# TrondVQ/UncertaintyQuantification-SleepApnea-1DCNN

Hardware: AMD Instinct MI355X
Metric: 30s-windows/sec for MCD T=50 & DE M=8 inference at 1/2/4/8 MI355X (higher is better)
Workload: dtype fp32; 1 GPU; global_batch=16384, seq_len=60, parallelism=dp1, mcd_passes=50, de_members=8, bn_mode_mcd=batch

## Files before the change

uncertaintyquantification_sleepapnea_1dcnn_amd/csrc/x3_api.h:

```cpp
#pragma once
#include <hip/hip_runtime_api.h>

#include <cstdint>

#include "x3_args.h"
#include "x3_geo.h"

namespace apneauq {
x3::LayerInfo x3_layer_info(int layer);
hipError_t x3_launch_layer(int layer, const x3::LayerArgs& A, int grid, bool dense_rows, hipStream_t stream);
hipError_t x3_launch_l1(const x3::L1Args& A, hipStream_t stream);
hipError_t x3_launch_aff(const x3::AffArgs& A, hipStream_t stream);
hipError_t x3_launch_head(const x3::HeadArgs& A, hipStream_t stream);
}
```

uncertaintyquantification_sleepapnea_1dcnn_amd/csrc/x3_bindings.cpp:

```cpp
#include "arch_tables.h"
#include "bind_util.h"
#include "x3_api.h"

namespace {
using namespace apneauq::bind;
constexpr auto& kCh = apneauq::arch::C;
constexpr auto& kKs = apneauq::arch::KS;

int num_cus(const at::Tensor& t) {
  int n = 0;
  check(hipDeviceGetAttribute(&n, hipDeviceAttributeMultiprocessorCount, t.device().index()), "hipDeviceGetAttribute");
  return n > 0 ? n : 256;
}

void x3_layer(int64_t layer, const at::Tensor& in, at::Tensor& out, const at::Tensor& wfrag, int64_t w_gstride,
              const at::Tensor& bias, const at::Tensor& wscale, int64_t p_gstride, const at::Tensor& aff_in,
              int64_t aff_gstride, const c10::optional<at::Tensor>& stats, int64_t n_win, int64_t groups,
              bool in_shared, int64_t thr_in, int64_t thr_out, int64_t seed, int64_t pass_base,
              int64_t window_offset, int64_t grid, const c10::optional<at::Tensor>& smax_in,
              const c10::optional<at::Tensor>& amax_in, const c10::optional<at::Tensor>& smax_out,
              const c10::optional<at::Tensor>& gscale_in, bool sign_in, bool sign_out, bool dense_rows) {
  TORCH_CHECK(layer >= 1 && layer <= 5, "x3_layer: layer must be 1..5 (block 2..6)");
  TORCH_CHECK(n_win >= 1 && groups >= 1, "x3_layer: empty launch");
  const int cin = kCh[layer], cout = kCh[layer + 1], ks = kKs[layer];
  const int64_t samples = n_win * groups, samples_in = in_shared ? n_win : samples;
  const apneauq::x3::LayerInfo info = apneauq::x3_layer_info((int)layer);
  TORCH_CHECK(!dense_rows || info.has_dense, "x3_layer: layer ", layer, " has no dense-row kernel");
  TORCH_CHECK(!dense_rows || n_win < (int64_t(1) << 24), "x3_layer: too many windows for dense rows");
  const int64_t tpg = apneauq::x3::tiles_per_group<int64_t>(dense_rows, n_win, info.S);
  TORCH_CHECK(tpg * groups < (int64_t(1) << 31), "x3_layer: too many tiles");
  const int64_t wgroups = w_gstride ? groups : 1, pgroups = p_gstride ? groups : 1;
  need(in, at::kFloat, samples_in * 60 * cin, "x3_layer: in");
  need(out, at::kFloat, layer == 5 ? samples * 2 * cout : samples * 60 * cout, "x3_layer: out");
  const int64_t frag = (int64_t)(cin / 32) * ks * (cout / 16) * 128;
  TORCH_CHECK(w_gstride == 0 || w_gstride == frag, "x3_layer: w_gstride must be 0 or ", frag);
  need(wfrag, at::kHalf, wgroups * frag * 8, "x3_layer: wfrag");
  TORCH_CHECK(p_gstride == 0 || p_gstride == cout, "x3_layer: p_gstride must be 0 or ", cout);
  need(bias, at::kFloat, pgroups * cout, "x3_layer: bias");
  need(wscale, at::kFloat, pgroups, "x3_layer: wscale");
  TORCH_CHECK(aff_gstride == 0 || aff_gstride == 2 * cin, "x3_layer: aff_gstride must be 0 or ", 2 * cin);
  need(aff_in, at::kFloat, (aff_gstride ? groups : 1) * 2 * cin, "x3_layer: aff_in");
  double* st = nullptr;
  if (stats.has_value()) {
// ... 39 lines not shown
  A.tiles_per_group = (int)tpg;
  A.total_tiles = (int)(tpg * groups);
  A.in_shared = in_shared ? 1 : 0;
  TORCH_CHECK(!(sign_in && in_shared), "x3_layer: the shared block-1 output carries no masks");
  TORCH_CHECK(!(sign_out && layer == 5), "x3_layer: block 6 reduces its masked output in place");
  A.sign_in = sign_in ? 1 : 0;
  A.sign_out = sign_out ? 1 : 0;
  A.thr_in = (unsigned)thr_in;
  A.thr_out = (unsigned)thr_out;
  A.layer = (int)layer;
  A.pass_base = (unsigned)pass_base;
  A.window_offset = (unsigned)window_offset;
  A.seed = (unsigned long long)seed;
  int g = grid > 0 ? (int)grid : num_cus(in) * info.WPC;
  if (g > A.total_tiles) g = A.total_tiles;
  check(apneauq::x3_launch_layer((int)layer, A, g, dense_rows, cur_stream()), "x3_layer");
}

void x3_l1(const at::Tensor& x, const at::Tensor& w, const at::Tensor& b, at::Tensor& out,
           const c10::optional<at::Tensor>& stats, int64_t n_win, int64_t groups, const c10::optional<at::Tensor>& smax) {
  TORCH_CHECK(n_win >= 1 && groups >= 1, "x3_l1: empty launch");
  need(x, at::kFloat, n_win * 60 * 4, "x3_l1: x");
  need(w, at::kFloat, groups * 7 * 4 * 128, "x3_l1: w");
  need(b, at::kFloat, groups * 128, "x3_l1: b");
  need(out, at::kFloat, groups * n_win * 60 * 128, "x3_l1: out");
  double* st = nullptr;
  if (stats.has_value()) {
    need(*stats, at::kDouble, groups * apneauq::x3::kStatSlots * 2 * 128, "x3_l1: stats");
    st = stats->data_ptr<double>();
  }
  unsigned* smp = nullptr;
// ... 55 lines not shown
  TORCH_CHECK(aff_gstride == 0 || aff_gstride == 2 * C, "x3_head: aff_gstride");
  TORCH_CHECK(p_gstride == 0 || p_gstride == C, "x3_head: p_gstride");
  need(sums, at::kFloat, samples * 2 * C, "x3_head: sums");
  need(aff, at::kFloat, (aff_gstride ? groups : 1) * 2 * C, "x3_head: aff");
  need(dw, at::kFloat, (p_gstride ? groups : 1) * C, "x3_head: dense w");
  need(db, at::kFloat, p_gstride ? groups : 1, "x3_head: dense b");
  need(out, at::kFloat, samples, "x3_head: out");
  const at::DeviceGuard guard(sums.device());
  apneauq::x3::HeadArgs A{sums.data_ptr<float>(), aff.data_ptr<float>(), dw.data_ptr<float>(), db.data_ptr<float>(),
                          out.data_ptr<float>(), C, (int)n_win, (int)samples, (int)aff_gstride, (int)p_gstride,
                          logits ? 1 : 0};
  check(apneauq::x3_launch_head(A, cur_stream()), "x3_head");
}

bool x3_has_dense(int64_t layer) { return apneauq::x3_layer_info((int)layer).has_dense; }

}

TORCH_LIBRARY_FRAGMENT(apneauq, m) {
  m.def("x3_layer(int layer, Tensor input, Tensor(a!) out, Tensor wfrag, int w_gstride, Tensor bias, Tensor wscale, "
        "int p_gstride, Tensor aff_in, int aff_gstride, Tensor(b!)? stats, int n_win, int groups, bool in_shared, "
        "int thr_in, int thr_out, int seed, int pass_base, int window_offset, int grid, Tensor? smax_in=None, "
        "Tensor? amax_in=None, Tensor(c!)? smax_out=None, Tensor? gscale_in=None, bool sign_in=False, bool sign_out=False, "
        "bool dense_rows=False) -> ()");
  m.def("x3_l1(Tensor x, Tensor w, Tensor b, Tensor(a!) out, Tensor(b!)? stats, int n_win, int groups, "
        "Tensor(c!)? smax=None) -> ()");
  m.def("x3_aff(Tensor? stats, Tensor gamma, Tensor beta, Tensor(a!) mmean, Tensor(b!) mvar, Tensor(c!) aff, int C, "
        "int groups, int p_gstride, bool update, int repeat, float inv_count, float eps, float momentum, float dsc, "
        "Tensor(d!)? amax=None, Tensor(e!)? gscale=None, bool running=False) -> ()");
  m.def("x3_head(Tensor sums, Tensor aff, int aff_gstride, Tensor dw, Tensor db, int p_gstride, Tensor(a!) out, "
        "int n_win, int groups, bool logits) -> ()");
  m.def("x3_has_dense(int layer) -> bool", &x3_has_dense);
}

TORCH_LIBRARY_IMPL(apneauq, CUDA, m) {
  m.impl("x3_layer", &x3_layer);
  m.impl("x3_l1", &x3_l1);
  m.impl("x3_head", &x3_head);
  m.impl("x3_aff", &x3_aff);
}
```

uncertaintyquantification_sleepapnea_1dcnn_amd/csrc/x3_geo.h:

```cpp
#pragma once

#include "x3_dense_map.h"

#ifndef __host__
#define APNEAUQ_X3_GEO_PLAIN 1
#define __host__
#define __device__
#endif

namespace apneauq {
namespace x3 {

constexpr int kStagers = 4;
constexpr int kL = 60, kSR = 64, kHalo = 4;
__host__ __device__ constexpr int row_bytes(int ck) { return 4 * ck + 32; }
__host__ __device__ constexpr int lds_rows(int S) { return kHalo + S * kSR + kHalo; }
__host__ __device__ constexpr int buf_bytes(int S, int ck) { return lds_rows(S) * row_bytes(ck); }
__host__ __device__ constexpr int tab_rows(int S, int ks) { return kSR * S + (ks - 1); }
__host__ __device__ constexpr int mask_tab_bytes(int S, int cout) { return kSR * S * (cout / 16) * 2; }
__host__ __device__ constexpr bool mask_tab_layer(int cin, int cout, int ks, int lw, bool dense_rows) {
  return dense_rows && lw > 0 && cin == 96 && cout == 256 && ks == 9;
}

template <int NW, int WPC>
constexpr int waves_per_eu() { return NW * WPC > 8 ? (NW * WPC + 3) / 4 : NW * WPC <= 4 ? 1 : 2; }
constexpr int loaders(int lw) { return lw > 0 ? lw : 0; }
constexpr int dense_lw(int lw, int wm, int wn) { return lw > 0 ? lw : -(wm * wn); }

struct Geo {
  int g, w0, wf, off, rows_left;
};

template <typename I>
__host__ __device__ constexpr I tiles_per_group(bool dense_rows, I n_win, int S) {
  return dense_rows ? (I)dense::tiles(n_win, kSR * S) : (n_win + S - 1) / S;
}
// ... 17 lines not shown
  static constexpr int kRowB = row_bytes(CK), NQ = CK / 32, kQ = CK / 4;
  static constexpr int PAD = (KS - 1) / 2, kRows = kSR * S;
  static_assert(!DENSE || (!PS && !LAST), "dense rows: batch-moment blocks 2..5 only");
  static_assert(kThreads <= 1024, "workgroup size");
  static constexpr int kBufB = DENSE ? dense::lds_rows(kRows) * kRowB : buf_bytes(S, CK);
  static constexpr int kValidRows = DENSE ? kRows : S * kL, kUnits = kValidRows * kQ;
  static constexpr int SW = LW > 0 ? LW : LW < 0 ? (-LW < NW ? -LW : NW) : (kStagers < NW ? kStagers : NW);
  static constexpr int kSBase = LW > 0 ? NWM * 64 : 0;
  static constexpr int kST = SW * 64;
  static constexpr int kMainU = (kUnits + kST - 1) / kST, kNU = kMainU + (DENSE ? 1 : 0);
  static constexpr int kEdgeWaves = (2 * PAD * kQ + 63) / 64;
  static_assert(!DENSE || (kUnits % kST == 0 && kEdgeWaves <= SW), "dense rows: whole staging steps per tile");
  static_assert(kST % kQ == 0 && (CK == 32 || CK == 64), "a staging thread keeps one channel quad");
  static constexpr int NCH = CIN / CK, NCTA = COUT / 16, NCT = NCTA / WN, NRT = 4 * S / WM;
  static constexpr int NSTEP = NCH * NQ * KS;
  static constexpr int RG = NCT >= 4                       ? 1
                            : (NCT >= 3 && NCT * NRT > 16) ? 1
                            : NCT == 1                     ? 4
                                                           : 2;
  static constexpr bool BDB = NCT * NRT <= 24 && RG < 4;
  static_assert(NRT % RG == 0, "row-tile groups");
  static constexpr long long FRAG_STEP = (long long)NCTA * 128;
  static_assert(CIN % CK == 0 && COUT % 16 == 0, "channel tiling");
  static_assert(NCTA % WN == 0 && (4 * S) % WM == 0, "wave tiling");
  static_assert(NRT % 4 == 0, "whole 64-row sample slots per wave row (epilogue keys, block 6 sums)");
  static_assert(S <= 8, "packed per-sample exponents");
  static constexpr int kSP = (S + 3) / 4;

  static constexpr int kTabRows = tab_rows(S, KS);
  static_assert(!DENSE || NCH >= 2, "row tables: a tile's tables are written one chunk of the same workgroup ahead");
  static constexpr bool kMaskTab = mask_tab_layer(CIN, COUT, KS, LW, DENSE);
  static constexpr int kMtRowW = COUT / 16, kMtT = kMaskTab ? kST / kRows : 1, kMtW = kMtRowW / kMtT;
  static constexpr int kMtPhase = (kMtW + (NCH > 1 ? NCH - 2 : 0)) / (NCH > 1 ? NCH - 1 : 1);
  static_assert(!kMaskTab || NCH >= 2, "mask table: written in the chunk iterations ahead of the tile's last");
  static_assert(!kMaskTab || (kST % kRows == 0 && kMtRowW % kMtT == 0), "mask table: whole words per loader thread");

// ... 28 lines not shown
#define APNEAUQ_X3_LAYERS(X)                            \
  X(1, 128, 192, 5, 4, 2, 4, false, -8, 0, 32, 1, true) \
  X(2, 192, 224, 3, 2, 1, 7, false, 4, 4, 64, 1, true)  \
  X(3, 224, 96, 7, 4, 2, 2, false, 4, 4, 32, 1, true)   \
  X(4, 96, 256, 9, 2, 1, 8, false, 4, 4, 32, 1, true)   \
  X(5, 256, 96, 9, 4, 2, 2, true, 4, 4, 64, 1, false)
#endif

namespace apneauq {
namespace x3 {

struct LayerInfo {
  int S, WPC;
  bool has_dense;
  int lds_ps, lds_batch, lds_dense;
};
template <bool HAVE, int CIN, int COUT, int KS, int S, int WM, int WN, int LW, int CK, int WPC>
constexpr int dense_lds_bytes() {
  if constexpr (HAVE) {
    return Cfg<CIN, COUT, KS, S, WM, WN, false, dense_lw(LW, WM, WN), CK, WPC, false, true>::bytes;
  } else {
    return 0;
  }
}
constexpr LayerInfo layer_info(int layer) {
#define APNEAUQ_X3_INFO(L, CI, CO, K, S, WM, WN, LAST, LW, LWB, CK, WPC, DENSE)                              \
  if (layer == L)                                                                                            \
    return LayerInfo{S, WPC, DENSE && !LAST, Cfg<CI, CO, K, S, WM, WN, LAST, LW, CK, WPC, true>::bytes,      \
                     Cfg<CI, CO, K, S, WM, WN, LAST, LWB, CK, WPC, false>::bytes,                            \
                     dense_lds_bytes<DENSE && !LAST, CI, CO, K, S, WM, WN, LWB, CK, WPC>()};
  APNEAUQ_X3_LAYERS(APNEAUQ_X3_INFO)
#undef APNEAUQ_X3_INFO
  return LayerInfo{0, 1, false, 0, 0, 0};
}

}
}

#ifdef APNEAUQ_X3_GEO_PLAIN
#undef __host__
#undef __device__
#undef APNEAUQ_X3_GEO_PLAIN
#endif
```

uncertaintyquantification_sleepapnea_1dcnn_amd/csrc/x3_layers.hip:

```cpp
#include "common.h"
#include "f16x3.h"
#include "x3_api.h"
#include "x3_dense_map.h"
#include "x3_geo.h"

namespace apneauq {
namespace x3 {

__device__ __forceinline__ int sample_prescale(unsigned rmax_bits, const float* amax) {
  return prescale_exp(__builtin_fmaf(amax[0], __uint_as_float(rmax_bits), amax[1]));
}

template <typename T>
__device__ __forceinline__ T gld(const void* p) {
  return *(const __attribute__((address_space(1))) T*)(p);
}

__device__ __forceinline__ int opaque_tid() {
  int t = threadIdx.x;
  asm volatile("" : "+v"(t));
  return t;
}

__device__ __forceinline__ void lds_barrier() {
  __builtin_amdgcn_fence(__ATOMIC_RELEASE, "workgroup", "local");
  __builtin_amdgcn_s_barrier();
  __builtin_amdgcn_fence(__ATOMIC_ACQUIRE, "workgroup", "local");
}

template <int CIN, int COUT, int KS, int S, int WM, int WN, bool LAST, int LW, int CK, int WPC, bool PS, bool DENSE = false>
__global__ __launch_bounds__((WM * WN + loaders(LW)) * 64, (waves_per_eu<WM * WN + loaders(LW), WPC>())) void layer_kernel(
    const LayerArgs A) {
  extern __shared__ __attribute__((aligned(16))) char smem[];
  using C = Cfg<CIN, COUT, KS, S, WM, WN, LAST, LW, CK, WPC, PS, DENSE>;
  constexpr int NWM = C::NWM, kThreads = C::kThreads, kCK = CK, kRowB = C::kRowB, NQ = C::NQ, kQ = C::kQ;
  constexpr int PAD = C::PAD, kRows = C::kRows, kS = S, kBufB = C::kBufB, kValidRows = C::kValidRows;
  constexpr int SW = C::SW, kSBase = C::kSBase, kST = C::kST, kMainU = C::kMainU, kNU = C::kNU;
  constexpr int NCH = C::NCH, NCT = C::NCT, NRT = C::NRT, NSTEP = C::NSTEP, RG = C::RG, kSP = C::kSP;
  constexpr bool BDB = C::BDB;
  constexpr long long FRAG_STEP = C::FRAG_STEP;
  constexpr int kTabRows = C::kTabRows;
  constexpr bool kMaskTab = C::kMaskTab;
  constexpr bool kBiasHoist = DENSE;
  constexpr int kMtRowW = C::kMtRowW, kMtT = C::kMtT, kMtW = C::kMtW, kMtPhase = C::kMtPhase;
  double* st = reinterpret_cast<double*>(smem + C::st);
  float* wsc = reinterpret_cast<float*>(smem + C::wsc);
  unsigned* ektab = reinterpret_cast<unsigned*>(smem + C::ektab);
  uint2* stab = reinterpret_cast<uint2*>(smem + C::stab);
  unsigned short* mtab = reinterpret_cast<unsigned short*>(smem + C::mtab);
// ... 405 lines not shown
            atomicAdd(&st[COUT + co0 + e], (double)b);
          }
        }
      }
    }
    if (track) {
#pragma unroll
      for (int q = 0; q < NRT / 4; ++q) {
        const float mq = wave_max(mxs[q]);
        const int w = w0 + (rt0 >> 2) + q;
        if (lane == 0 && w < A.n_win) atomicMax(A.smax_out + (long long)g * A.n_win + w, __float_as_uint(mq));
      }
    }
  };

  auto flush_stats = [&](int g) {
    __syncthreads();
    if (A.stats != nullptr) {
      double* dst = A.stats + ((long long)g * kStatSlots + slot) * 2 * COUT;
      for (int i = DENSE ? opaque_tid() : tid; i < 2 * COUT; i += kThreads) {
        atomicAdd(dst + i, st[i]);
        st[i] = 0.0;
      }
    }
    __syncthreads();
  };

  for (int i = tid; i < C::st / 16; i += kThreads) reinterpret_cast<f32x4*>(smem)[i] = f32x4{0.f, 0.f, 0.f, 0.f};
  for (int i = tid; i < 2 * COUT; i += kThreads) st[i] = 0.0;
  if (DENSE && stager) write_tables(t_begin);
// ... 21 lines not shown
      if (stager && total > 1) load_chunk(chunk_tile(1), 1 % NCH, s0);
#pragma unroll 1
      for (int it = 0; it < total; ++it) {
        const int tile = chunk_tile(it), c = it - (tile - t_begin) * NCH;
        group_change(tile, c);
        if (stager && it + 1 < total) store_chunk(chunk_tile(it + 1), (it + 1) % NCH, smem + ((it + 1) & 1) * kBufB, s0);
        if (kMaskTab && stager && mask_out && c < NCH - 1) draw_mask(tile, c);
        lds_barrier();
        if (stager && it + 2 < total) load_chunk(chunk_tile(it + 2), (it + 2) % NCH, s0);
      }
      flush_stats(g_cur);
      return;
    }
    lds_barrier();
    load_a(wbase(t_begin), ah, al);
#pragma unroll 1
    for (int it = 0; it < total; ++it) {
      const int tile = chunk_tile(it), c = it - (tile - t_begin) * NCH;
      group_change(tile, c);
      const gf16x8* wcur = wbase(tile);
      const gf16x8* wnxt = wbase(tile + 1 < t_end ? tile + 1 : tile);
      compute_chunk(c, tile_off(tile), smem + (it & 1) * kBufB, wcur, wnxt, []() {});
      if (c == NCH - 1) epilogue(tile);
      lds_barrier();
    }
    flush_stats(g_cur);
    return;
  }
  if (stager) {
    load_chunk(t_begin, 0, s0);
// ... 167 lines not shown
  const long long sidx = (long long)blockIdx.x * 4 + (threadIdx.x >> 6);
  if (sidx >= A.samples) return;
  const int g = (int)(sidx / A.n_win);
  const float* s = A.sums + sidx * 2 * A.C;
  const float* af = A.aff + (long long)g * A.aff_gstride;
  const float* dw = A.dw + (long long)g * A.p_gstride;
  float v = 0.f;
  for (int c = lane; c < A.C; c += 64) v += dw[c] * __builtin_fmaf(af[c], s[c], af[A.C + c] * s[A.C + c]);
  v = wave_sum(v);
  if (lane == 0) {
    const float logit = v * (1.0f / kL) + A.db[A.p_gstride ? g : 0];
    A.out[sidx] = A.out_logits ? logit : 1.0f / (1.0f + expf(-logit));
  }
}

template <int CIN, int COUT, int KS, int S, int WM, int WN, bool LAST, int LW, int CK, int WPC, bool PS, bool DENSE = false>
hipError_t launch_layer(const LayerArgs& A, int grid, hipStream_t stream) {
  using C = Cfg<CIN, COUT, KS, S, WM, WN, LAST, LW, CK, WPC, PS, DENSE>;
  auto k = layer_kernel<CIN, COUT, KS, S, WM, WN, LAST, LW, CK, WPC, PS, DENSE>;
  static bool attr = false;
  if (!attr) {
    hipError_t e = hipFuncSetAttribute(reinterpret_cast<const void*>(k), hipFuncAttributeMaxDynamicSharedMemorySize, C::bytes);
    if (e != hipSuccess) return e;
    attr = true;
  }
  hipLaunchKernelGGL(k, dim3(grid), dim3(C::kThreads), C::bytes, stream, A);
  return hipGetLastError();
}

template <bool HAVE, int CIN, int COUT, int KS, int S, int WM, int WN, int LW, int CK, int WPC>
hipError_t launch_dense(const LayerArgs& A, int grid, hipStream_t stream) {
  if constexpr (HAVE) {
    return launch_layer<CIN, COUT, KS, S, WM, WN, false, dense_lw(LW, WM, WN), CK, WPC, false, true>(A, grid, stream);
  } else {
    return hipErrorInvalidValue;
  }
}

}

x3::LayerInfo x3_layer_info(int layer) { return x3::layer_info(layer); }

hipError_t x3_launch_layer(int layer, const x3::LayerArgs& A, int grid, bool dense_rows, hipStream_t stream) {
  using namespace x3;
  const bool ps = A.smax_in != nullptr || A.smax_out != nullptr;
#define APNEAUQ_X3_LAUNCH(L, CI, CO, K, S, WM, WN, LAST, LW, LWB, CK, WPC, DENSE)                                  \
  if (layer == L) {                                                                                       \
    if (dense_rows)                                                                                       \
      return ps ? hipErrorInvalidValue                                                                    \
                : launch_dense<DENSE && !LAST, CI, CO, K, S, WM, WN, LWB, CK, WPC>(A, grid, stream);       \
    return ps ? launch_layer<CI, CO, K, S, WM, WN, LAST, LW, CK, WPC, true>(A, grid, stream)               \
              : launch_layer<CI, CO, K, S, WM, WN, LAST, LWB, CK, WPC, false>(A, grid, stream);            \
  }
  APNEAUQ_X3_LAYERS(APNEAUQ_X3_LAUNCH)
#undef APNEAUQ_X3_LAUNCH
  return hipErrorInvalidValue;
}

hipError_t x3_launch_l1(const x3::L1Args& A, hipStream_t stream) {
  const int grid = A.groups * A.blocks_per_group;
  if (grid <= 0) return hipSuccess;
  hipLaunchKernelGGL(x3::l1_kernel, dim3(grid), dim3(256), 0, stream, A);
  return hipGetLastError();
}

// ... 14 lines not shown
```

uncertaintyquantification_sleepapnea_1dcnn_amd/ops/x3.py:

```python
from __future__ import annotations

import math
import os
from typing import Callable, Dict, List, Optional, Sequence

import torch

from ..models.spec import ModelSpec
from . import _ext, fused, rng

CH = fused.FUSED_CHANNELS
KS = fused.FUSED_KSIZES
STAT_SLOTS = 16
CK = 32
BYTES_PER_SAMPLE = 60 * (192 + 256) * 4
R1_BYTES = 60 * 128 * 4


def supports(spec: ModelSpec) -> bool:
    return fused.supports(spec)


def pack_conv(kernel: torch.Tensor):
    k, cin, cout = kernel.shape
# ... 114 lines not shown

def set_dense_layers(layers: Optional[Sequence[int]]) -> Optional[frozenset]:
    global _dense_override
    prev = _dense_override
    _dense_override = None if layers is None else frozenset(int(l) for l in layers)
    return prev


def _dense_layers() -> frozenset:
    if _dense_override is not None:
        return _dense_override
    v = os.environ.get("APNEAUQ_X3_DENSE", _DENSE_DEFAULT)
    return frozenset(int(t) for t in v.replace(" ", "").split(",") if t)


def _dsc(rate: float) -> float:
    return 1.0 / (1.0 - rate) if rate < 1.0 else 0.0


def _sync_stats(sync: Callable, st: torch.Tensor, groups: int, c: int) -> None:
    v = st[: groups * STAT_SLOTS * 2 * c].view(groups, STAT_SLOTS, 2 * c)
    tot = v.sum(1)
    sync(tot)
    v.zero_()
    v[:, 0].copy_(tot)


def _max_samples(dev, per_sample: int, frac: float = 0.45) -> int:
    free = torch.cuda.mem_get_info(dev)[0]
    cap = float(os.environ.get("APNEAUQ_X3_WS_GB", "20")) * 2 ** 30
    return max(1, int(min(free * frac, cap)) // per_sample)


def _layer(model: X3Model, ws: "_Workspace", l: int, *, n: int, groups: int, dropout: bool, stats=None,
           shared_r1: bool = False, pass_affines: bool = False, seed: int = 0, pass_base: int = 0,
           window_offset: int = 0, grid: int = 0, prescale: str = "group", sign: frozenset = frozenset(),
           dense: frozenset = frozenset()) -> None:
    per_member = model.G > 1
    src = ws.r1 if l == 1 else ws.buf[(l - 2) % 2]
    dst = ws.sums if l == 5 else ws.buf[(l - 1) % 2]
    thr = [rng.dropout_threshold(model.spec.blocks[i].dropout) if dropout else 0 for i in (l - 1, l)]
    if prescale == "sample":
        pre = (ws.smax[l - 1], ws.amax[l - 1], ws.smax_out(l, groups * n), None)
    else:
        pre = (None, None, None, ws.gscale[l - 1])
    _ops().x3_layer(l, src, dst, model.wfrag[l], model.wfrag[l].shape[1] // 8 if per_member else 0, model.bias[l],
                    model.wscale[l], CH[l + 1] if per_member else 0, ws.aff[l - 1],
                    2 * CH[l] if per_member or (pass_affines and l > 1) else 0, stats, n, groups,
                    bool(shared_r1 and l == 1), *thr, int(seed) & ((1 << 63) - 1), int(pass_base), int(window_offset),
                    int(grid), *pre, *_sign(l, sign), l in dense)


def _aff(model: X3Model, ws: "_Workspace", l: int, *, groups: int, dropout: bool, stats=None, update: bool = False,
         repeat: int = 1, inv_count: float = 1.0, amax: bool = False, gscale: bool = False,
         running: bool = False) -> None:
    g, b, mm, mv = model.bn[l]
    _ops().x3_aff(stats, g, b, mm, mv, ws.aff[l], CH[l + 1], groups, CH[l + 1] if model.G > 1 else 0, bool(update),
                  repeat, inv_count, float(model.spec.bn_epsilon), float(model.spec.bn_momentum),
                  _dsc(model.spec.blocks[l].dropout) if dropout else 1.0, ws.amax[l] if amax else None,
                  ws.gscale[l] if gscale else None, running)


def _head(model: X3Model, ws: "_Workspace", *, n: int, groups: int, pass_affines: bool = False, logits: bool = False):
    per_member = model.G > 1
    _ops().x3_head(ws.sums, ws.aff[5], 2 * CH[6] if per_member or pass_affines else 0, model.dw, model.db,
# ... 21 lines not shown
            max_samples = int(t.item())
    ref_n = n
    if sync is not None and global_n:
        import torch.distributed as dist

        w = dist.get_world_size() if dist.is_initialized() else 1
        ref_n = -(-gn // w)
    if ref_n > max_samples:
        return _mcd_batch_windowed(model, x, n_pass, seed, pass_base, window_offset, update_moving, sync, gn,
                                   max_samples)
    cap = max(1, min(n_pass, max_samples // max(ref_n, 1)))
    n_chunks = -(-n_pass // cap)
    chunk = -(-n_pass // n_chunks)
    ws = model.workspace(chunk * n, n, chunk)
    inv_count = 1.0 / (gn * 60.0)
    sl, dl = _sign_layers(), _dense_layers()
    out = torch.empty(n_pass, n, dtype=torch.float32, device=model.device)
    ws.stats[0].zero_()
    o.x3_l1(x, model.w1, model.b1, ws.r1, ws.stats[0], n, 1, None)
    if sync is not None:
        _sync_stats(sync, ws.stats[0], 1, CH[1])
    _aff(model, ws, 0, groups=1, dropout=True, stats=ws.stats[0], update=update_moving, repeat=n_pass,
         inv_count=inv_count, gscale=True)
    for t0 in range(0, n_pass, chunk):
        tc = min(chunk, n_pass - t0)
        for l in range(1, 6):
            c = CH[l + 1]
            st = ws.stats[l]
            st[: tc * STAT_SLOTS * 2 * c].zero_()
            _layer(model, ws, l, n=n, groups=tc, dropout=True, stats=st, shared_r1=True, pass_affines=True, seed=seed,
                   pass_base=int(pass_base) + t0, window_offset=window_offset, grid=grid, sign=sl, dense=dl)
            if sync is not None:
                _sync_stats(sync, st, tc, c)
            _aff(model, ws, l, groups=tc, dropout=True, stats=st, update=update_moving, inv_count=inv_count,
                 gscale=True)
        _head(model, ws, n=n, groups=tc, pass_affines=True)
        out[t0: t0 + tc].copy_(ws.out[: tc * n].view(tc, n))
    return out


def _mcd_batch_windowed(model: X3Model, x: torch.Tensor, n_pass: int, seed: int, pass_base: int,
                        window_offset: int, update_moving: bool, sync: Optional[Callable], gn: int,
                        max_samples: int) -> torch.Tensor:
    o = _ops()
    n = x.shape[0]
    wc = max(1, int(max_samples))
    bounds = [(s, min(n, s + wc)) for s in range(0, n, wc)]
    ws = model.workspace(wc, wc, 1)
    inv_count = 1.0 / (gn * 60.0)
    sl, dl = _sign_layers(), _dense_layers()
    out = torch.empty(n_pass, n, dtype=torch.float32, device=model.device)

    def run(s: int, e: int, upto: int, pb: int, stats_layer: int) -> None:
        m = e - s
        o.x3_l1(x[s:e], model.w1, model.b1, ws.r1, ws.stats[0] if stats_layer == 0 else None, m, 1, None)
        for l in range(1, upto + 1):
            _layer(model, ws, l, n=m, groups=1, dropout=True, stats=ws.stats[l] if l == stats_layer else None,
                   shared_r1=True, pass_affines=True, seed=seed, pass_base=pb, window_offset=int(window_offset) + s,
                   sign=sl, dense=dl)

    def finish_layer(l: int, repeat: int) -> None:
        if sync is not None:
            _sync_stats(sync, ws.stats[l], 1, CH[l + 1])
        _aff(model, ws, l, groups=1, dropout=True, stats=ws.stats[l], update=update_moving, repeat=repeat,
             inv_count=inv_count, gscale=True)

    ws.stats[0].zero_()
    for s, e in bounds:
        run(s, e, 0, int(pass_base), 0)
    finish_layer(0, n_pass)
    for t in range(n_pass):
        pb = int(pass_base) + t
        for l in range(1, 6):
            ws.stats[l].zero_()
# ... 43 lines not shown
        _layer(model, ws, l, n=n, groups=groups, dropout=dropout, shared_r1=dropout, seed=seed, pass_base=pass_offset,
               window_offset=window_offset, prescale="sample", sign=sl)
    if features:
        if groups != 1:
            raise ValueError("features of one model and one pass")
        sums = ws.sums[: n * 2 * CH[6]].view(n, 2, CH[6])
        aff = ws.aff[5][: 2 * CH[6]].view(2, CH[6])
        return (aff[0] * sums[:, 0] + aff[1] * sums[:, 1]) / 60.0
    _head(model, ws, n=n, groups=groups, logits=logits)
    return ws.out[: groups * n].view(G, n_pass, n).clone()


def _predict_members(model: X3Model, ws: "_Workspace", x: torch.Tensor, G: int, logits: bool) -> torch.Tensor:
    o = _ops()
    n = x.shape[0]
    dl = _dense_layers()
    o.zero_buffers([ws.stats[l][: G * STAT_SLOTS * 2 * CH[l + 1]] for l in range(5)])
    _aff(model, ws, 5, groups=G, dropout=False)
    o.x3_l1(x, model.w1, model.b1, ws.r1, ws.stats[0], n, G, None)
    for l in range(1, 6):
        _aff(model, ws, l - 1, groups=G, dropout=False, stats=ws.stats[l - 1], gscale=True, running=True)
        _layer(model, ws, l, n=n, groups=G, dropout=False, stats=ws.stats[l] if l < 5 else None, dense=dl)
    _head(model, ws, n=n, groups=G, logits=logits)
    return ws.out[: G * n].view(G, 1, n).clone()


@torch.no_grad()
def features_running(model: X3Model, x: torch.Tensor, max_samples: Optional[int] = None) -> torch.Tensor:
    if model.G != 1:
        raise ValueError("features of one model")
    x = x.to(device=model.device, dtype=torch.float32).contiguous()
    n = x.shape[0]
    if n == 0:
        return torch.empty(0, CH[6], dtype=torch.float32, device=model.device)
    if max_samples is None:
        max_samples = _max_samples(model.device, BYTES_PER_SAMPLE + R1_BYTES)
    wc = max(1, int(max_samples))
# ... 23 lines not shown
```

Measured before the change: 67350 windows/s.

## Overlap layer-3 epilogue with final-chunk MFMA compute in dense-row kernel

Adds an OVL variant of the dense-row layer kernel for the 224->96, k=7 layer (layer 3 by default). The last input-channel chunk's MFMA work is split into two phases by output-channel tile, so the epilogue of the first part (bias, ReLU, dropout masks, stats, stores) can run while the MFMAs of the second part are still issuing. The aim is to hide epilogue latency behind tensor-core work. In exchange it adds code complexity and more register pressure, which could lower occupancy.

```diff
diff --git a/uncertaintyquantification_sleepapnea_1dcnn_amd/csrc/x3_api.h b/uncertaintyquantification_sleepapnea_1dcnn_amd/csrc/x3_api.h
--- a/uncertaintyquantification_sleepapnea_1dcnn_amd/csrc/x3_api.h
+++ b/uncertaintyquantification_sleepapnea_1dcnn_amd/csrc/x3_api.h
@@ -8,7 +8,7 @@
 
 namespace apneauq {
 x3::LayerInfo x3_layer_info(int layer);
-hipError_t x3_launch_layer(int layer, const x3::LayerArgs& A, int grid, bool dense_rows, hipStream_t stream);
+hipError_t x3_launch_layer(int layer, const x3::LayerArgs& A, int grid, bool dense_rows, bool overlap, hipStream_t stream);
 hipError_t x3_launch_l1(const x3::L1Args& A, hipStream_t stream);
 hipError_t x3_launch_aff(const x3::AffArgs& A, hipStream_t stream);
 hipError_t x3_launch_head(const x3::HeadArgs& A, hipStream_t stream);
diff --git a/uncertaintyquantification_sleepapnea_1dcnn_amd/csrc/x3_bindings.cpp b/uncertaintyquantification_sleepapnea_1dcnn_amd/csrc/x3_bindings.cpp
--- a/uncertaintyquantification_sleepapnea_1dcnn_amd/csrc/x3_bindings.cpp
+++ b/uncertaintyquantification_sleepapnea_1dcnn_amd/csrc/x3_bindings.cpp
@@ -19,7 +19,8 @@
               bool in_shared, int64_t thr_in, int64_t thr_out, int64_t seed, int64_t pass_base,
               int64_t window_offset, int64_t grid, const c10::optional<at::Tensor>& smax_in,
               const c10::optional<at::Tensor>& amax_in, const c10::optional<at::Tensor>& smax_out,
-              const c10::optional<at::Tensor>& gscale_in, bool sign_in, bool sign_out, bool dense_rows) {
+              const c10::optional<at::Tensor>& gscale_in, bool sign_in, bool sign_out, bool dense_rows,
+              bool overlap) {
   TORCH_CHECK(layer >= 1 && layer <= 5, "x3_layer: layer must be 1..5 (block 2..6)");
   TORCH_CHECK(n_win >= 1 && groups >= 1, "x3_layer: empty launch");
   const int cin = kCh[layer], cout = kCh[layer + 1], ks = kKs[layer];
@@ -27,6 +28,7 @@
   const apneauq::x3::LayerInfo info = apneauq::x3_layer_info((int)layer);
   TORCH_CHECK(!dense_rows || info.has_dense, "x3_layer: layer ", layer, " has no dense-row kernel");
   TORCH_CHECK(!dense_rows || n_win < (int64_t(1) << 24), "x3_layer: too many windows for dense rows");
+  TORCH_CHECK(!overlap || (dense_rows && info.overlap != apneauq::x3::kOvlNone), "x3_layer: layer ", layer, " has no epilogue-overlap kernel");
   const int64_t tpg = apneauq::x3::tiles_per_group<int64_t>(dense_rows, n_win, info.S);
   TORCH_CHECK(tpg * groups < (int64_t(1) << 31), "x3_layer: too many tiles");
   const int64_t wgroups = w_gstride ? groups : 1, pgroups = p_gstride ? groups : 1;
@@ -96,7 +98,7 @@
   A.seed = (unsigned long long)seed;
   int g = grid > 0 ? (int)grid : num_cus(in) * info.WPC;
   if (g > A.total_tiles) g = A.total_tiles;
-  check(apneauq::x3_launch_layer((int)layer, A, g, dense_rows, cur_stream()), "x3_layer");
+  check(apneauq::x3_launch_layer((int)layer, A, g, dense_rows, overlap, cur_stream()), "x3_layer");
 }
 
 void x3_l1(const at::Tensor& x, const at::Tensor& w, const at::Tensor& b, at::Tensor& out,
@@ -182,6 +184,7 @@
 }
 
 bool x3_has_dense(int64_t layer) { return apneauq::x3_layer_info((int)layer).has_dense; }
+int64_t x3_overlap_kind(int64_t layer) { return apneauq::x3_layer_info((int)layer).overlap; }
 
 }
 
@@ -190,7 +193,7 @@
         "int p_gstride, Tensor aff_in, int aff_gstride, Tensor(b!)? stats, int n_win, int groups, bool in_shared, "
         "int thr_in, int thr_out, int seed, int pass_base, int window_offset, int grid, Tensor? smax_in=None, "
         "Tensor? amax_in=None, Tensor(c!)? smax_out=None, Tensor? gscale_in=None, bool sign_in=False, bool sign_out=False, "
-        "bool dense_rows=False) -> ()");
+        "bool dense_rows=False, bool overlap=False) -> ()");
   m.def("x3_l1(Tensor x, Tensor w, Tensor b, Tensor(a!) out, Tensor(b!)? stats, int n_win, int groups, "
         "Tensor(c!)? smax=None) -> ()");
   m.def("x3_aff(Tensor? stats, Tensor gamma, Tensor beta, Tensor(a!) mmean, Tensor(b!) mvar, Tensor(c!) aff, int C, "
@@ -199,6 +202,7 @@
   m.def("x3_head(Tensor sums, Tensor aff, int aff_gstride, Tensor dw, Tensor db, int p_gstride, Tensor(a!) out, "
         "int n_win, int groups, bool logits) -> ()");
   m.def("x3_has_dense(int layer) -> bool", &x3_has_dense);
+  m.def("x3_overlap_kind(int layer) -> int", &x3_overlap_kind);
 }
 
 TORCH_LIBRARY_IMPL(apneauq, CUDA, m) {
diff --git a/uncertaintyquantification_sleepapnea_1dcnn_amd/csrc/x3_geo.h b/uncertaintyquantification_sleepapnea_1dcnn_amd/csrc/x3_geo.h
--- a/uncertaintyquantification_sleepapnea_1dcnn_amd/csrc/x3_geo.h
+++ b/uncertaintyquantification_sleepapnea_1dcnn_amd/csrc/x3_geo.h
@@ -20,6 +20,24 @@
 __host__ __device__ constexpr int mask_tab_bytes(int S, int cout) { return kSR * S * (cout / 16) * 2; }
 __host__ __device__ constexpr bool mask_tab_layer(int cin, int cout, int ks, int lw, bool dense_rows) {
   return dense_rows && lw > 0 && cin == 96 && cout == 256 && ks == 9;
+}
+
+constexpr int kOvlNone = 0, kOvlChan = 1, kOvlRow = 2;
+struct Overlap {
+  int kind, point;
+};
+__host__ __device__ constexpr Overlap overlap_layer(int cin, int cout, int ks, int lw, bool dense_rows) {
+  if (!dense_rows) return Overlap{kOvlNone, 0};
+  if (cin == 224 && cout == 96 && ks == 7 && lw > 0) return Overlap{kOvlChan, 1};
+  return Overlap{kOvlNone, 0};
+}
+__host__ __device__ constexpr int row_group(int nct, int nrt) {
+  return nct >= 4 ? 1 : (nct >= 3 && nct * nrt > 16) ? 1 : nct == 1 ? 4 : 2;
+}
+__host__ __device__ constexpr bool b_double_buffer(int nct, int nrt) { return nct * nrt <= 24 && row_group(nct, nrt) < 4; }
+__host__ __device__ constexpr int part_lo(int kind, int point, int axis, int p) { return p == 0 || kind != axis ? 0 : point; }
+__host__ __device__ constexpr int part_hi(int kind, int point, int axis, int p, int n) {
+  return p == 0 && kind == axis ? point : n;
 }
 
 template <int NW, int WPC>
@@ -67,12 +85,32 @@
   static_assert(kST % kQ == 0 && (CK == 32 || CK == 64), "a staging thread keeps one channel quad");
   static constexpr int NCH = CIN / CK, NCTA = COUT / 16, NCT = NCTA / WN, NRT = 4 * S / WM;
   static constexpr int NSTEP = NCH * NQ * KS;
-  static constexpr int RG = NCT >= 4                       ? 1
-                            : (NCT >= 3 && NCT * NRT > 16) ? 1
-                            : NCT == 1                     ? 4
-                                                           : 2;
-  static constexpr bool BDB = NCT * NRT <= 24 && RG < 4;
+  static constexpr int RG = row_group(NCT, NRT);
+  static constexpr bool BDB = b_double_buffer(NCT, NRT);
   static_assert(NRT % RG == 0, "row-tile groups");
+  static constexpr int kOvlKind = overlap_layer(CIN, COUT, KS, LW, DENSE).kind;
+  static constexpr int kOvlPoint = overlap_layer(CIN, COUT, KS, LW, DENSE).point;
+  static constexpr int kNK = NQ * KS;
+  static constexpr int kOvlCT1 = kOvlKind == kOvlChan ? kOvlPoint : NCT, kOvlRT1 = kOvlKind == kOvlRow ? kOvlPoint : NRT;
+  static constexpr int kOvlN1 = kOvlKind == kOvlNone ? 0 : kOvlCT1 * kOvlRT1;
+  static constexpr int kOvlSlots = kNK > 1 ? kNK - 1 : 1;
+  __host__ __device__ static constexpr int ovl_ct_lo(int p) { return part_lo(kOvlKind, kOvlPoint, kOvlChan, p); }
+  __host__ __device__ static constexpr int ovl_ct_hi(int p) { return part_hi(kOvlKind, kOvlPoint, kOvlChan, p, NCT); }
+  __host__ __device__ static constexpr int ovl_rt_lo(int p) { return part_lo(kOvlKind, kOvlPoint, kOvlRow, p); }
+  __host__ __device__ static constexpr int ovl_rt_hi(int p) { return part_hi(kOvlKind, kOvlPoint, kOvlRow, p, NRT); }
+  __host__ __device__ static constexpr int ovl_tile_ct(int i) { return i / kOvlRT1; }
+  __host__ __device__ static constexpr int ovl_tile_rt(int i) { return i % kOvlRT1; }
+  __host__ __device__ static constexpr int ovl_slot(int i) { return i * kOvlSlots / (kOvlN1 > 0 ? kOvlN1 : 1); }
+  __host__ __device__ static constexpr int ovl_rg(int p) {
+    return ovl_ct_hi(p) - ovl_ct_lo(p) == 1 ? 2 : row_group(ovl_ct_hi(p) - ovl_ct_lo(p), ovl_rt_hi(p) - ovl_rt_lo(p));
+  }
+  __host__ __device__ static constexpr bool ovl_bdb(int p) {
+    return (ovl_ct_hi(p) - ovl_ct_lo(p)) * (ovl_rt_hi(p) - ovl_rt_lo(p)) <= 24 && ovl_rg(p) < 4;
+  }
+  static_assert(kOvlKind == kOvlNone || (DENSE && kOvlPoint > 0 && kOvlPoint < (kOvlKind == kOvlChan ? NCT : NRT)),
+                "epilogue overlap: a dense-row kernel, both parts non-empty");
+  static_assert(kOvlKind == kOvlNone || (kOvlRT1 % 2 == 0 && (NRT - kOvlRT1) % 2 == 0),
+                "epilogue overlap: whole row-tile groups (1 or 2) per phase");
   static constexpr long long FRAG_STEP = (long long)NCTA * 128;
   static_assert(CIN % CK == 0 && COUT % 16 == 0, "channel tiling");
   static_assert(NCTA % WN == 0 && (4 * S) % WM == 0, "wave tiling");
@@ -131,6 +169,7 @@
   int S, WPC;
   bool has_dense;
   int lds_ps, lds_batch, lds_dense;
+  int overlap;
 };
 template <bool HAVE, int CIN, int COUT, int KS, int S, int WM, int WN, int LW, int CK, int WPC>
 constexpr int dense_lds_bytes() {
@@ -140,15 +179,24 @@
     return 0;
   }
 }
+template <bool HAVE, int CIN, int COUT, int KS, int S, int WM, int WN, int LW, int CK, int WPC>
+constexpr int dense_overlap_kind() {
+  if constexpr (HAVE) {
+    return Cfg<CIN, COUT, KS, S, WM, WN, false, dense_lw(LW, WM, WN), CK, WPC, false, true>::kOvlKind;
+  } else {
+    return kOvlNone;
+  }
+}
 constexpr LayerInfo layer_info(int layer) {
 #define APNEAUQ_X3_INFO(L, CI, CO, K, S, WM, WN, LAST, LW, LWB, CK, WPC, DENSE)                              \
   if (layer == L)                                                                                            \
     return LayerInfo{S, WPC, DENSE && !LAST, Cfg<CI, CO, K, S, WM, WN, LAST, LW, CK, WPC, true>::bytes,      \
                      Cfg<CI, CO, K, S, WM, WN, LAST, LWB, CK, WPC, false>::bytes,                            \
-                     dense_lds_bytes<DENSE && !LAST, CI, CO, K, S, WM, WN, LWB, CK, WPC>()};
+                     dense_lds_bytes<DENSE && !LAST, CI, CO, K, S, WM, WN, LWB, CK, WPC>(),                  \
+                     dense_overlap_kind<DENSE && !LAST, CI, CO, K, S, WM, WN, LWB, CK, WPC>()};
   APNEAUQ_X3_LAYERS(APNEAUQ_X3_INFO)
 #undef APNEAUQ_X3_INFO
-  return LayerInfo{0, 1, false, 0, 0, 0};
+  return LayerInfo{0, 1, false, 0, 0, 0, kOvlNone};
 }
 
 }
diff --git a/uncertaintyquantification_sleepapnea_1dcnn_amd/csrc/x3_layers.hip b/uncertaintyquantification_sleepapnea_1dcnn_amd/csrc/x3_layers.hip
--- a/uncertaintyquantification_sleepapnea_1dcnn_amd/csrc/x3_layers.hip
+++ b/uncertaintyquantification_sleepapnea_1dcnn_amd/csrc/x3_layers.hip
@@ -1,3 +1,5 @@
+#include <type_traits>
+
 #include "common.h"
 #include "f16x3.h"
 #include "x3_api.h"
@@ -28,11 +30,23 @@
   __builtin_amdgcn_fence(__ATOMIC_ACQUIRE, "workgroup", "local");
 }
 
-template <int CIN, int COUT, int KS, int S, int WM, int WN, bool LAST, int LW, int CK, int WPC, bool PS, bool DENSE = false>
+typedef unsigned u32x4 __attribute__((ext_vector_type(4)));
+
+template <int B, int E, typename F>
+__device__ __forceinline__ void static_for(F&& f) {
+  if constexpr (B < E) {
+    f(std::integral_constant<int, B>{});
+    static_for<B + 1, E>(f);
+  }
+}
+
+template <int CIN, int COUT, int KS, int S, int WM, int WN, bool LAST, int LW, int CK, int WPC, bool PS, bool DENSE = false,
+          bool OVL = false>
 __global__ __launch_bounds__((WM * WN + loaders(LW)) * 64, (waves_per_eu<WM * WN + loaders(LW), WPC>())) void layer_kernel(
     const LayerArgs A) {
   extern __shared__ __attribute__((aligned(16))) char smem[];
   using C = Cfg<CIN, COUT, KS, S, WM, WN, LAST, LW, CK, WPC, PS, DENSE>;
+  static_assert(!OVL || (C::kOvlKind != kOvlNone && LW > 0), "epilogue overlap: a layer overlap_layer() splits");
   constexpr int NWM = C::NWM, kThreads = C::kThreads, kCK = CK, kRowB = C::kRowB, NQ = C::NQ, kQ = C::kQ;
   constexpr int PAD = C::PAD, kRows = C::kRows, kS = S, kBufB = C::kBufB, kValidRows = C::kValidRows;
   constexpr int SW = C::SW, kSBase = C::kSBase, kST = C::kST, kMainU = C::kMainU, kNU = C::kNU;
@@ -468,6 +482,183 @@
     }
   };
 
+  auto compute_phase = [&](auto ph, int off, const char* buf, const gf16x8* wcur, const gf16x8* wnxt, auto&& hook) {
+    if constexpr (OVL) {
+      constexpr int P = decltype(ph)::value;
+      constexpr int CL = C::ovl_ct_lo(P), CH = C::ovl_ct_hi(P), RL = C::ovl_rt_lo(P), RH = C::ovl_rt_hi(P);
+      constexpr int PRG = C::ovl_rg(P), kNK = C::kNK;
+      constexpr bool PBDB = C::ovl_bdb(P);
+      const char* bp[NRT];
+#pragma unroll
+      for (int rt = RL; rt < RH; ++rt)
+        bp[rt] = buf + bofs + (off + (dense::kSlot - kL) * ((off + (rt0 + rt) * 16 + m) / kL)) * kRowB;
+      const gf16x8* wk = wcur + (long long)(NCH - 1) * kNK * FRAG_STEP;
+      asm volatile("" : "+v"(wk));
+      static_for<0, kNK>([&](auto kk_) {
+        constexpr int kk = decltype(kk_)::value, q2 = kk / KS, j = kk - q2 * KS;
+        constexpr bool last = kk + 1 == kNK;
+        constexpr int B_CL = C::ovl_ct_lo(1), B_CH = C::ovl_ct_hi(1);
+        constexpr int LL = !last ? CL : P == 0 ? (CL > B_CL ? CL : B_CL) : 0;
+        constexpr int LH = !last ? CH : P == 0 ? (CH < B_CH ? CH : B_CH) : NCT;
+        const gf16x8* np = !last ? wk + (long long)(kk + 1) * FRAG_STEP : P == 0 ? wk : wnxt;
+        f16x8 nh[NCT], nl[NCT];
+#pragma unroll
+        for (int ct = LL; ct < LH; ++ct) {
+          nh[ct] = np[ct * 128];
+          nl[ct] = np[ct * 128 + 64];
+        }
+        __builtin_amdgcn_sched_barrier(0);
+        auto ldb = [&](int rt, f16x8& h_, f16x8& l_) {
+          const char* br = bp[rt] + q2 * 64;
+          h_ = *reinterpret_cast<const f16x8*>(br + (rt * 16 + j) * kRowB);
+          l_ = *reinterpret_cast<const f16x8*>(br + (rt * 16 + j) * kRowB + 2 * kCK);
+        };
+        f16x8 bh[PRG], bl[PRG];
+#pragma unroll
+        for (int r = 0; r < PRG; ++r) ldb(RL + r, bh[r], bl[r]);
+#pragma unroll
+        for (int rg = RL; rg < RH; rg += PRG) {
+          f16x8 bh2[PRG], bl2[PRG];
+#pragma unroll
+          for (int r = 0; r < PRG; ++r) {
+            bh2[r] = bh[r];
+            bl2[r] = bl[r];
+            if (PBDB && rg + PRG < RH) ldb(rg + PRG + r, bh2[r], bl2[r]);
+            if (!PBDB) ldb(rg + r, bh[r], bl[r]);
+          }
+          __builtin_amdgcn_sched_barrier(0);
+#pragma unroll
+          for (int r = 0; r < PRG; ++r)
+#pragma unroll
+            for (int ct = CL; ct < CH; ++ct) acc[ct][rg + r] = mfma(ah[ct], bh[r], acc[ct][rg + r]);
+#pragma unroll
+          for (int r = 0; r < PRG; ++r)
+#pragma unroll
+            for (int ct = CL; ct < CH; ++ct) acc[ct][rg + r] = mfma(al[ct], bh[r], acc[ct][rg + r]);
+#pragma unroll
+          for (int r = 0; r < PRG; ++r)
+#pragma unroll
+            for (int ct = CL; ct < CH; ++ct) acc[ct][rg + r] = mfma(ah[ct], bl[r], acc[ct][rg + r]);
+#pragma unroll
+          for (int r = 0; r < PRG; ++r) {
+            bh[r] = bh2[r];
+            bl[r] = bl2[r];
+          }
+        }
+#pragma unroll
+        for (int ct = LL; ct < LH; ++ct) {
+          ah[ct] = nh[ct];
+          al[ct] = nl[ct];
+        }
+        __builtin_amdgcn_sched_barrier(0);
+        hook(kk_);
+      });
+    }
+  };
+  struct Ovl {
+    float wsq;
+    f32x4 bq[NCT];
+    f32x4 s1, s2;
+    __amdgpu_buffer_rsrc_t out;
+    int voff;
+    int rel0;
+    int rows_left;
+  };
+  auto ovl_begin = [&](int tile, Ovl& o_) {
+    if constexpr (OVL) {
+      const int lane = opaque_tid() & 63, m = lane & 15, h = lane >> 4;
+      const Geo G = tile_geo(tile);
+      o_.wsq = wsc[(tile & 1) * kS];
+      const float* bias = A.bias + (long long)G.g * A.p_gstride + ct0 * 16 + 4 * h;
+#pragma unroll
+      for (int ct = 0; ct < NCT; ++ct) o_.bq[ct] = gld<f32x4>(bias + ct * 16);
+      o_.rel0 = rt0 * 16 + m;
+      o_.rows_left = G.rows_left < kRows ? G.rows_left : kRows;
+      float* base = A.out + ((long long)G.g * A.n_win * kL + G.w0) * COUT;
+      o_.out = __builtin_amdgcn_make_buffer_rsrc(base, 0, o_.rows_left * COUT * 4, 0x00020000);
+      o_.voff = (o_.rel0 * COUT + ct0 * 16 + 4 * h) * 4;
+    }
+  };
+  auto ovl_slice = [&](int tile, Ovl& o_, auto ct_, auto rt_, bool first, bool last) {
+    if constexpr (OVL) {
+      constexpr int ct = decltype(ct_)::value, rt = decltype(rt_)::value;
+      const int h = (opaque_tid() & 63) >> 4;
+      f32x4 r;
+#pragma unroll
+      for (int e = 0; e < 4; ++e) r[e] = fmaxf(__builtin_fmaf(acc[ct][rt][e], o_.wsq, o_.bq[ct][e]), 0.f);
+      acc[ct][rt] = f32x4{0.f, 0.f, 0.f, 0.f};
+      bool keep[4] = {true, true, true, true};
+      unsigned sgn = 0u;
+      if constexpr (kMaskTab) {
+        if (mask_out) sgn = ~((unsigned)mtab[(o_.rel0 + rt * 16) * kMtRowW + ct0 + ct] >> (4 * h));
+      } else if (mask_out) {
+        const unsigned kt = ektab[(tile & 1) * kRows + o_.rel0 + rt * 16];
+        const unsigned cp = (unsigned)((ct0 + ct) * 16 + 4 * h) >> 1;
+        const unsigned b01 = mix32(kt ^ cp), b23 = mix32(kt ^ (cp + 1u));
+        keep[0] = (b01 & 0xFFFFu) >= A.thr_out;
+        keep[1] = (b01 >> 16) >= A.thr_out;
+        keep[2] = (b23 & 0xFFFFu) >= A.thr_out;
+        keep[3] = (b23 >> 16) >= A.thr_out;
+      }
+      if (first) o_.s1 = o_.s2 = f32x4{0.f, 0.f, 0.f, 0.f};
+      if (o_.rows_left < kRows) {
+        const bool valid = o_.rel0 + rt * 16 < o_.rows_left;
+#pragma unroll
+        for (int e = 0; e < 4; ++e) r[e] = valid ? r[e] : 0.f;
+      }
+#pragma unroll
+      for (int e = 0; e < 4; ++e) {
+        o_.s1[e] += r[e];
+        o_.s2[e] = __builtin_fmaf(r[e], r[e], o_.s2[e]);
+      }
+      f32x4 o = r;
+      if constexpr (kMaskTab) {
+#pragma unroll
+        for (int e = 0; e < 4; ++e) o[e] = __uint_as_float(__float_as_uint(r[e]) | ((sgn << (31 - e)) & 0x80000000u));
+      } else if (mask_out) {
+#pragma unroll
+        for (int e = 0; e < 4; ++e) o[e] = keep[e] ? r[e] : __builtin_copysignf(r[e], -1.f);
+      }
+      __builtin_amdgcn_raw_buffer_store_b128(__builtin_bit_cast(u32x4, o), o_.out, o_.voff + (rt * 16 * COUT + ct * 16) * 4, 0, 0);
+      if (last && A.stats != nullptr) {
+        const int m = opaque_tid() & 15, co0 = (ct0 + ct) * 16 + 4 * h;
+#pragma unroll
+        for (int e = 0; e < 4; ++e) {
+          const float a = group16_sum(o_.s1[e]), b = group16_sum(o_.s2[e]);
+          if (m == 0) {
+            atomicAdd(&st[co0 + e], (double)a);
+            atomicAdd(&st[COUT + co0 + e], (double)b);
+          }
+        }
+      }
+    }
+  };
+  auto overlap_chunk = [&](int tile, int off, const char* buf, const gf16x8* wcur, const gf16x8* wnxt, auto&& hook) {
+    if constexpr (OVL) {
+      constexpr int RT1 = C::kOvlRT1;
+      Ovl o_;
+      ovl_begin(tile, o_);
+      compute_phase(std::integral_constant<int, 0>{}, off, buf, wcur, wnxt, [&](auto kk_) {
+        if constexpr (decltype(kk_)::value == C::kNK / 2) hook();
+      });
+      compute_phase(std::integral_constant<int, 1>{}, off, buf, wcur, wnxt, [&](auto kk_) {
+        static_for<0, C::kOvlN1>([&](auto i_) {
+          constexpr int i = decltype(i_)::value, rt = C::ovl_tile_rt(i);
+          constexpr bool first = rt == 0, last = rt == RT1 - 1;
+          if constexpr (C::ovl_slot(i) == decltype(kk_)::value)
+            ovl_slice(tile, o_, std::integral_constant<int, C::ovl_tile_ct(i)>{}, std::integral_constant<int, rt>{}, first, last);
+        });
+        __builtin_amdgcn_sched_barrier(0);
+      });
+      static_for<C::ovl_ct_lo(1), C::ovl_ct_hi(1)>([&](auto ct_) {
+        static_for<C::ovl_rt_lo(1), C::ovl_rt_hi(1)>([&](auto rt_) {
+          constexpr int rt = decltype(rt_)::value;
+          constexpr bool first = rt == C::ovl_rt_lo(1), last = rt == C::ovl_rt_hi(1) - 1;
+          ovl_slice(tile, o_, ct_, rt_, first, last);
+        });
+      });
+    }
+  };
   auto flush_stats = [&](int g) {
     __syncthreads();
     if (A.stats != nullptr) {
@@ -519,6 +710,26 @@
     }
     lds_barrier();
     load_a(wbase(t_begin), ah, al);
+    if constexpr (OVL) {
+      int it = 0;
+#pragma unroll 1
+      for (int tile = t_begin; tile < t_end; ++tile) {
+        group_change(tile, 0);
+        const gf16x8* wcur = wbase(tile);
+        const gf16x8* wnxt = wbase(tile + 1 < t_end ? tile + 1 : tile);
+        const int off = tile_off(tile);
+#pragma unroll 1
+        for (int c = 0; c < NCH - 1; ++c, ++it) {
+          compute_chunk(c, off, smem + (it & 1) * kBufB, wcur, wnxt, []() {});
+          lds_barrier();
+        }
+        overlap_chunk(tile, off, smem + (it & 1) * kBufB, wcur, wnxt, []() {});
+        lds_barrier();
+        ++it;
+      }
+      flush_stats(g_cur);
+      return;
+    }
 #pragma unroll 1
     for (int it = 0; it < total; ++it) {
       const int tile = chunk_tile(it), c = it - (tile - t_begin) * NCH;
@@ -716,10 +927,11 @@
   }
 }
 
-template <int CIN, int COUT, int KS, int S, int WM, int WN, bool LAST, int LW, int CK, int WPC, bool PS, bool DENSE = false>
+template <int CIN, int COUT, int KS, int S, int WM, int WN, bool LAST, int LW, int CK, int WPC, bool PS, bool DENSE = false,
+          bool OVL = false>
 hipError_t launch_layer(const LayerArgs& A, int grid, hipStream_t stream) {
   using C = Cfg<CIN, COUT, KS, S, WM, WN, LAST, LW, CK, WPC, PS, DENSE>;
-  auto k = layer_kernel<CIN, COUT, KS, S, WM, WN, LAST, LW, CK, WPC, PS, DENSE>;
+  auto k = layer_kernel<CIN, COUT, KS, S, WM, WN, LAST, LW, CK, WPC, PS, DENSE, OVL>;
   static bool attr = false;
   if (!attr) {
     hipError_t e = hipFuncSetAttribute(reinterpret_cast<const void*>(k), hipFuncAttributeMaxDynamicSharedMemorySize, C::bytes);
@@ -731,26 +943,29 @@
 }
 
 template <bool HAVE, int CIN, int COUT, int KS, int S, int WM, int WN, int LW, int CK, int WPC>
-hipError_t launch_dense(const LayerArgs& A, int grid, hipStream_t stream) {
+hipError_t launch_dense(const LayerArgs& A, int grid, bool overlap, hipStream_t stream) {
   if constexpr (HAVE) {
-    return launch_layer<CIN, COUT, KS, S, WM, WN, false, dense_lw(LW, WM, WN), CK, WPC, false, true>(A, grid, stream);
-  } else {
-    return hipErrorInvalidValue;
-  }
+    constexpr int lw = dense_lw(LW, WM, WN);
+    if (!overlap) return launch_layer<CIN, COUT, KS, S, WM, WN, false, lw, CK, WPC, false, true>(A, grid, stream);
+    if constexpr (Cfg<CIN, COUT, KS, S, WM, WN, false, lw, CK, WPC, false, true>::kOvlKind != kOvlNone)
+      return launch_layer<CIN, COUT, KS, S, WM, WN, false, lw, CK, WPC, false, true, true>(A, grid, stream);
+  }
+  return hipErrorInvalidValue;
 }
 
 }
 
 x3::LayerInfo x3_layer_info(int layer) { return x3::layer_info(layer); }
 
-hipError_t x3_launch_layer(int layer, const x3::LayerArgs& A, int grid, bool dense_rows, hipStream_t stream) {
+hipError_t x3_launch_layer(int layer, const x3::LayerArgs& A, int grid, bool dense_rows, bool overlap, hipStream_t stream) {
   using namespace x3;
   const bool ps = A.smax_in != nullptr || A.smax_out != nullptr;
+  if (overlap && !dense_rows) return hipErrorInvalidValue;
 #define APNEAUQ_X3_LAUNCH(L, CI, CO, K, S, WM, WN, LAST, LW, LWB, CK, WPC, DENSE)                                  \
   if (layer == L) {                                                                                       \
     if (dense_rows)                                                                                       \
       return ps ? hipErrorInvalidValue                                                                    \
-                : launch_dense<DENSE && !LAST, CI, CO, K, S, WM, WN, LWB, CK, WPC>(A, grid, stream);       \
+                : launch_dense<DENSE && !LAST, CI, CO, K, S, WM, WN, LWB, CK, WPC>(A, grid, overlap, stream); \
     return ps ? launch_layer<CI, CO, K, S, WM, WN, LAST, LW, CK, WPC, true>(A, grid, stream)               \
               : launch_layer<CI, CO, K, S, WM, WN, LAST, LWB, CK, WPC, false>(A, grid, stream);            \
   }
diff --git a/uncertaintyquantification_sleepapnea_1dcnn_amd/ops/x3.py b/uncertaintyquantification_sleepapnea_1dcnn_amd/ops/x3.py
--- a/uncertaintyquantification_sleepapnea_1dcnn_amd/ops/x3.py
+++ b/uncertaintyquantification_sleepapnea_1dcnn_amd/ops/x3.py
@@ -152,6 +152,24 @@
     return frozenset(int(t) for t in v.replace(" ", "").split(",") if t)
 
 
+_OVERLAP_DEFAULT = "3"
+_overlap_override: Optional[frozenset] = None
+
+
+def set_overlap_layers(layers: Optional[Sequence[int]]) -> Optional[frozenset]:
+    global _overlap_override
+    prev = _overlap_override
+    _overlap_override = None if layers is None else frozenset(int(l) for l in layers)
+    return prev
+
+
+def _overlap_layers() -> frozenset:
+    if _overlap_override is not None:
+        return _overlap_override
+    v = os.environ.get("APNEAUQ_X3_OVERLAP", _OVERLAP_DEFAULT)
+    return frozenset(int(t) for t in v.replace(" ", "").split(",") if t)
+
+
 def _dsc(rate: float) -> float:
     return 1.0 / (1.0 - rate) if rate < 1.0 else 0.0
 
@@ -173,7 +191,7 @@
 def _layer(model: X3Model, ws: "_Workspace", l: int, *, n: int, groups: int, dropout: bool, stats=None,
            shared_r1: bool = False, pass_affines: bool = False, seed: int = 0, pass_base: int = 0,
            window_offset: int = 0, grid: int = 0, prescale: str = "group", sign: frozenset = frozenset(),
-           dense: frozenset = frozenset()) -> None:
+           dense: frozenset = frozenset(), overlap: frozenset = frozenset()) -> None:
     per_member = model.G > 1
     src = ws.r1 if l == 1 else ws.buf[(l - 2) % 2]
     dst = ws.sums if l == 5 else ws.buf[(l - 1) % 2]
@@ -186,7 +204,7 @@
                     model.wscale[l], CH[l + 1] if per_member else 0, ws.aff[l - 1],
                     2 * CH[l] if per_member or (pass_affines and l > 1) else 0, stats, n, groups,
                     bool(shared_r1 and l == 1), *thr, int(seed) & ((1 << 63) - 1), int(pass_base), int(window_offset),
-                    int(grid), *pre, *_sign(l, sign), l in dense)
+                    int(grid), *pre, *_sign(l, sign), l in dense, l in dense and l in overlap)
 
 
 def _aff(model: X3Model, ws: "_Workspace", l: int, *, groups: int, dropout: bool, stats=None, update: bool = False,
@@ -238,7 +256,7 @@
     chunk = -(-n_pass // n_chunks)
     ws = model.workspace(chunk * n, n, chunk)
     inv_count = 1.0 / (gn * 60.0)
-    sl, dl = _sign_layers(), _dense_layers()
+    sl, dl, ol = _sign_layers(), _dense_layers(), _overlap_layers()
     out = torch.empty(n_pass, n, dtype=torch.float32, device=model.device)
     ws.stats[0].zero_()
     o.x3_l1(x, model.w1, model.b1, ws.r1, ws.stats[0], n, 1, None)
@@ -253,7 +271,7 @@
             st = ws.stats[l]
             st[: tc * STAT_SLOTS * 2 * c].zero_()
             _layer(model, ws, l, n=n, groups=tc, dropout=True, stats=st, shared_r1=True, pass_affines=True, seed=seed,
-                   pass_base=int(pass_base) + t0, window_offset=window_offset, grid=grid, sign=sl, dense=dl)
+                   pass_base=int(pass_base) + t0, window_offset=window_offset, grid=grid, sign=sl, dense=dl, overlap=ol)
             if sync is not None:
                 _sync_stats(sync, st, tc, c)
             _aff(model, ws, l, groups=tc, dropout=True, stats=st, update=update_moving, inv_count=inv_count,
@@ -272,7 +290,7 @@
     bounds = [(s, min(n, s + wc)) for s in range(0, n, wc)]
     ws = model.workspace(wc, wc, 1)
     inv_count = 1.0 / (gn * 60.0)
-    sl, dl = _sign_layers(), _dense_layers()
+    sl, dl, ol = _sign_layers(), _dense_layers(), _overlap_layers()
     out = torch.empty(n_pass, n, dtype=torch.float32, device=model.device)
 
     def run(s: int, e: int, upto: int, pb: int, stats_layer: int) -> None:
@@ -281,7 +299,7 @@
         for l in range(1, upto + 1):
             _layer(model, ws, l, n=m, groups=1, dropout=True, stats=ws.stats[l] if l == stats_layer else None,
                    shared_r1=True, pass_affines=True, seed=seed, pass_base=pb, window_offset=int(window_offset) + s,
-                   sign=sl, dense=dl)
+                   sign=sl, dense=dl, overlap=ol)
 
     def finish_layer(l: int, repeat: int) -> None:
         if sync is not None:
@@ -355,13 +373,13 @@
 def _predict_members(model: X3Model, ws: "_Workspace", x: torch.Tensor, G: int, logits: bool) -> torch.Tensor:
     o = _ops()
     n = x.shape[0]
-    dl = _dense_layers()
+    dl, ol = _dense_layers(), _overlap_layers()
     o.zero_buffers([ws.stats[l][: G * STAT_SLOTS * 2 * CH[l + 1]] for l in range(5)])
     _aff(model, ws, 5, groups=G, dropout=False)
     o.x3_l1(x, model.w1, model.b1, ws.r1, ws.stats[0], n, G, None)
     for l in range(1, 6):
         _aff(model, ws, l - 1, groups=G, dropout=False, stats=ws.stats[l - 1], gscale=True, running=True)
-        _layer(model, ws, l, n=n, groups=G, dropout=False, stats=ws.stats[l] if l < 5 else None, dense=dl)
+        _layer(model, ws, l, n=n, groups=G, dropout=False, stats=ws.stats[l] if l < 5 else None, dense=dl, overlap=ol)
     _head(model, ws, n=n, groups=G, logits=logits)
     return ws.out[: G * n].view(G, 1, n).clone()
 
```

Result: no change. 67400 windows/s, median of 6 (+0.1%).
